# damien911224/ZeroShotVideoClassification

Hardware: AMD Instinct MI355X
Metric: clips/sec (fwd+bwd+step) R(2+1)D-18 16x112x112 bs=22/GPU (higher is better)
Workload: dtype f32; 1 GPU; r2plus1d_18 training step (zero_grad+fwd+MSE+bwd+Adam), 22 clips/GPU 3x16x112x112, random-init, fp32 (BASELINE.json configs[1]); clips_per_gpu=22, global_batch=22, optimizer=Adam lr=1e-3 (torch.optim.Adam), parallelism=dp1, world_size=1, launcher=single process, input=resident

## Files before the change

zeroshotvideoclassification_amd/csrc/conv_params.h:

```cpp
#pragma once
#include <hip/hip_runtime.h>
#include <stdint.h>
#include "zsv_hip.h"
#include "zsv_common.h"

namespace zsv {

struct IgemmParams {
    int M;
    int P;
    int K;
    int taps, nHW, nW, nT, nH;
    int cS, cHW, cW;
    int oS, oHW, oW;
    int stT, stH, stW, rT, rH, rW;
    int gC, gT, gH, gW, gS, gHW;
    int gsT, gsH, gsW, goT, goH, goW;
    int dir;
    int a_m_stride, a_c_stride;
    int k0T, k0H, k0W, tsT, tsH, tsW, kH, kW;
    unsigned g_bytes, a_bytes;
    int relu;
    int ksplit;
    int slab_elems;
    int lds_epilogue;
    float* stat_sum;
    float* stat_sq;
    int tiles_n;
    const float* pre_coef;
    int pre_pitch;
    int t2_cin;
    const float* acc_src;
};

inline bool t2_dense_shape(const zsv_conv_desc* d) {
    return d->kT == 3 && d->kH == 1 && d->kW == 1 && d->sT == 1 && d->sH == 1 && d->sW == 1 && d->pT == 1 && d->pH == 0 &&
           d->pW == 0 && d->Ti == 2 && d->To == 2 && d->Cin >= 16 && d->Cout >= 16;
}
inline zsv_conv_desc t2_dense_desc(const zsv_conv_desc* d) {
    zsv_conv_desc e = *d;
    e.Cin = 2 * d->Cin; e.Cout = 2 * d->Cout;
    e.Ti = e.To = 1; e.kT = 1; e.pT = 0;
    return e;
}
__host__ __device__ inline long t2_weight_offset(int co2, int c2, int cin) {
    return ((long)(co2 >> 1) * cin + (c2 >> 1)) * 3 + ((c2 & 1) - (co2 & 1) + 1);
}

enum { PANEL_NONE = 0, PANEL_LAUNCH_ONLY = 2, PANEL_RECORD = 3, PANEL_QUERY = 4 };
struct PanelCtx {
    int mode;
    void* ptr;
    size_t bytes;
    size_t need;
    int jobs;
    zsv_pack_job job;
};
extern thread_local PanelCtx g_panel;
inline bool panel_stop() { return g_panel.mode == PANEL_RECORD || g_panel.mode == PANEL_QUERY; }
inline bool panel_place(size_t need, void* workspace, float*& panel, int& st) {
    PanelCtx& pc = g_panel;
    st = ZSV_OK;
    panel = (float*)workspace;
    if (pc.mode == PANEL_QUERY) { pc.need = need; pc.jobs++; return false; }
    if (pc.mode != PANEL_NONE) {
        if (!pc.ptr || pc.bytes < need || (reinterpret_cast<uintptr_t>(pc.ptr) & 15) != 0) { st = ZSV_E_WORKSPACE; return false; }
        panel = (float*)pc.ptr;
    }
    return true;
}

template <int X> struct LdPad { static constexpr int value = (X % 32 == 16) ? X : X + 16; };

__device__ __forceinline__ int sgpr(int v) { return __builtin_amdgcn_readfirstlane(v); }


template <int TM, int TN>
__device__ __forceinline__ void store_tiles(const IgemmParams& prm, const f32x4 (&acc)[TM][TN], int m_base, int p_base,
                                            int lane, const float* __restrict__ bias, float* __restrict__ C) {
    const int frag_row = lane >> 4, frag_col = lane & 15;
#pragma unroll
    for (int j = 0; j < TN; ++j) {
        const int p = p_base + 16 * j + frag_col;
        if (p >= prm.P) continue;
        const int n = p / prm.cS;
        int r = p - n * prm.cS;
        const int ct = r / prm.cHW;
        r -= ct * prm.cHW;
        const int chh = r / prm.cW;
        const int cw = r - chh * prm.cW;
        const int sp = (ct * prm.stT + prm.rT) * prm.oHW + (chh * prm.stH + prm.rH) * prm.oW + cw * prm.stW + prm.rW;
        float* cbase = C + (size_t)n * prm.M * prm.oS + sp;
#pragma unroll
        for (int i = 0; i < TM; ++i) {
#pragma unroll
            for (int r4 = 0; r4 < 4; ++r4) {
                const int m = m_base + 16 * i + 4 * frag_row + r4;
                if (m < prm.M) {
                    float v = acc[i][j][r4];
                    if (prm.acc_src != nullptr) v += prm.acc_src[(cbase - C) + (size_t)m * prm.oS];
                    if (bias != nullptr) v += bias[m];
                    if (prm.relu) v = fmaxf(v, 0.f);
                    cbase[(size_t)m * prm.oS] = v;
                }
            }
        }
    }
}

template <int TM, int TN, int WGM, int WGN>
__device__ __forceinline__ void store_tiles_lds(const IgemmParams& prm, const f32x4 (&acc)[TM][TN], float* cs, int cap,
                                                int m0, int n0, int wave, int lane, const float* __restrict__ bias,
                                                float* __restrict__ C) {
    constexpr int BM = 16 * TM * WGM;
    constexpr int BN = 16 * TN * WGN;
    constexpr int PITCH = BN + 4;
    constexpr int RPI = 256 / BN == 0 ? 1 : 256 / BN;
    static_assert(BN == 128 || BN == 256, "read-back assumes 32 or 64 float4 per row");
    const int wm0 = (wave / WGN) * (16 * TM);
    const int wn0 = (wave % WGN) * (16 * TN);
    const int frag_row = lane >> 4, frag_col = lane & 15;
    int rp = (cap / PITCH) & ~15;
    if (rp > BM) rp = BM;
    const int c4 = BN == 128 ? (lane & 31) : lane;
    const int rsub = BN == 128 ? (lane >> 5) : 0;
    for (int r0 = 0; r0 < BM; r0 += rp) {
        __syncthreads();
#pragma unroll
        for (int i = 0; i < TM; ++i) {
            const int rb = wm0 + 16 * i - r0;
            if (rb >= 0 && rb < rp) {
#pragma unroll
                for (int j = 0; j < TN; ++j)
#pragma unroll
                    for (int r = 0; r < 4; ++r)
                        cs[(rb + 4 * frag_row + r) * PITCH + wn0 + 16 * j + frag_col] = acc[i][j][r];
            }
        }
        __syncthreads();
        const int rows = min(rp, BM - r0);
        const int p = n0 + 4 * c4;
        const bool pvalid = p < prm.P;
        const int n = pvalid ? p / prm.cS : 0;
        float* cbase = C + (size_t)n * prm.M * prm.oS + (p - n * prm.cS);
        f32x4 addn = {0.f, 0.f, 0.f, 0.f};
        auto fetch_add = [&](int rr) {
            const int m = m0 + r0 + rr;
            addn = f32x4{0.f, 0.f, 0.f, 0.f};
            if (pvalid && m < prm.M) addn = *reinterpret_cast<const f32x4*>(prm.acc_src + (cbase - C) + (size_t)m * prm.oS);
        };
        const bool has_add = prm.acc_src != nullptr;
        if (has_add && wave * RPI + rsub < rows) fetch_add(wave * RPI + rsub);
        for (int rr = wave * RPI + rsub; rr < rows; rr += 4 * RPI) {
            const int m = m0 + r0 + rr;
            f32x4 v = *reinterpret_cast<const f32x4*>(&cs[rr * PITCH + 4 * c4]);
            if (has_add) {
                v += addn;
                if (rr + 4 * RPI < rows) fetch_add(rr + 4 * RPI);
            }
            if (prm.stat_sum != nullptr) {
                float s1 = (v[0] + v[1]) + (v[2] + v[3]);
                float s2 = (v[0] * v[0] + v[1] * v[1]) + (v[2] * v[2] + v[3] * v[3]);
#pragma unroll
                for (int o = (BN == 128 ? 16 : 32); o > 0; o >>= 1) {
                    s1 += __shfl_xor(s1, o, 64);
                    s2 += __shfl_xor(s2, o, 64);
                }
                if (c4 == 0 && m < prm.M) {
                    const int tn = n0 / BN;
                    prm.stat_sum[(size_t)m * prm.tiles_n + tn] = s1;
                    prm.stat_sq[(size_t)m * prm.tiles_n + tn] = s2;
                }
            }
            if (pvalid && m < prm.M) {
                if (bias != nullptr) { const float b = bias[m]; v[0] += b; v[1] += b; v[2] += b; v[3] += b; }
                if (prm.relu) { v[0] = fmaxf(v[0], 0.f); v[1] = fmaxf(v[1], 0.f); v[2] = fmaxf(v[2], 0.f); v[3] = fmaxf(v[3], 0.f); }
                *reinterpret_cast<f32x4*>(cbase + (size_t)m * prm.oS) = v;
            }
        }
    }
}

__device__ __forceinline__ int xcd_tile(int nwg, int bid) {
    const int q = nwg >> 3, r = nwg & 7, xcd = bid & 7;
    return (xcd < r ? xcd * (q + 1) : r * (q + 1) + (xcd - r) * q) + (bid >> 3);
}

int igemm_generic(const IgemmParams& prm, bool avec, const float* A, const float* G, const float* bias, float* C,
                  hipStream_t stream);
bool igemm_tap_applicable(const IgemmParams& prm);
size_t igemm_tap_workspace_bytes(const IgemmParams& prm);
int igemm_tap(const IgemmParams& prm, const float* W, int w_m_stride, int w_c_stride, const float* G,
              const float* bias, float* C, void* workspace, size_t workspace_bytes, float* slabs, hipStream_t stream);
int igemm_tap_ksplit(const IgemmParams& prm);
int igemm_tap_stat_tiles(const IgemmParams& prm, const float* C);
int splitk_reduce(const float* slabs, int ksplit, long elems, int M, int oS, const float* bias, int relu, float* C,
                  hipStream_t stream);
int conv_check(const zsv_conv_desc* d);
size_t wgrad_generic_workspace_bytes(const zsv_conv_desc* d);
int wgrad_generic(const zsv_conv_desc* d, const float* x, const float* dy, float* dw, void* workspace,
                  size_t workspace_bytes, hipStream_t stream);
bool wino_dgrad_applicable(const zsv_conv_desc* d);
size_t wino_dgrad_workspace_bytes(const zsv_conv_desc* d);
int wino_dgrad(const zsv_conv_desc* d, const float* dy, const float* w, const float* add, float* dx, void* workspace,
               size_t workspace_bytes, hipStream_t stream);
bool dgrad_s2_applicable(const zsv_conv_desc* d);
size_t dgrad_s2_workspace_bytes(const zsv_conv_desc* d);
bool dgrad_s2_sub_supported(const zsv_conv_desc* d, int st, int sh, int sw);
int dgrad_s2(const zsv_conv_desc* d, const float* dy, const float* w, const float* sub, int sub_st, float* dx, void* workspace,
             size_t workspace_bytes, hipStream_t stream);
bool wino_fwd_applicable(const zsv_conv_desc* d);
bool wino_fwd_pre_capable(const zsv_conv_desc* d);
int wino_fwd_pre(const zsv_conv_desc* d, const float* x, const float* pre_coef, int pre_pitch, const float* w, float* stat_sum,
                 float* stat_sq, float* y, void* workspace, size_t workspace_bytes, hipStream_t stream);
bool wino_fwd_fusable(const zsv_conv_desc* d);
bool wino_dgrad_fusable(const zsv_conv_desc* d);
int wino_fwd_stat_tiles(const zsv_conv_desc* d);
size_t wino_fwd_workspace_bytes(const zsv_conv_desc* d);
int wino_fwd(const zsv_conv_desc* d, const float* x, const float* w, const float* bias, const float* residual, int relu,
             float* stat_sum, float* stat_sq, float* y, void* workspace, size_t workspace_bytes, hipStream_t stream);
bool wgrad_dma_applicable(const zsv_conv_desc* d, const float* x, const float* dy);
size_t wgrad_dma_workspace_bytes(const zsv_conv_desc* d);
int wgrad_dma(const zsv_conv_desc* d, const float* x, const float* dy, void* workspace, size_t workspace_bytes,
              int* slices_out, int* cpad_out, hipStream_t stream, const unsigned* vm_ext = nullptr);
int wgrad_vmask(const zsv_conv_desc* d, unsigned* out, hipStream_t stream);
bool wgrad_tring_applicable(const zsv_conv_desc* d, const float* x, const float* dy);
size_t wgrad_tring_workspace_bytes(const zsv_conv_desc* d);
int wgrad_tring_pre(const zsv_conv_desc* d, const float* x, const float* pre_coef, int pre_pitch, const float* dy, float* dw,
                    void* workspace, size_t workspace_bytes, hipStream_t stream);
int wgrad_tring(const zsv_conv_desc* d, const float* x, const float* dy, float* dw, void* workspace, size_t workspace_bytes,
                hipStream_t stream);
bool wgrad_wino_applicable(const zsv_conv_desc* d, const float* x, const float* dy);
size_t wgrad_wino_workspace_bytes(const zsv_conv_desc* d);
int wgrad_wino(const zsv_conv_desc* d, const float* x, const float* dy, float* dw, void* workspace, size_t workspace_bytes,
               hipStream_t stream, const unsigned* vm_ext = nullptr);

}
```

zeroshotvideoclassification_amd/csrc/conv_wgrad.hip:

```cpp
#include <hip/hip_runtime.h>
#include <stdint.h>
#include <stdlib.h>
#include "conv_params.h"
#include "knobs.h"

namespace zsv {

typedef float f32x2 __attribute__((ext_vector_type(2)));

struct WgradParams {
    int M;
    int Cin, Cpad, nblk;
    int taps, kHW, kW;
    int Kp;
    int P;
    int oS, oHW, oW;
    Magic m_oS, m_oHW, m_oW;
    int gT, gH, gW, gS, gHW, gCS;
    int sT, sH, sW, pT, pH, pW;
    int chunks_per_slice;
    unsigned x_bytes, dy_bytes;
};

template <int TM, int TN, int WGM, int WGN, bool AV4, int BP, bool TWOTAP>
__global__ __launch_bounds__(256, (BP == 16 ? 3 : 2)) void conv_wgrad_kernel(WgradParams prm, const float* __restrict__ X,
                                                         const float* __restrict__ DY,
                                                         float* __restrict__ OUT, int tiles_m, int tiles_mn) {
    constexpr int BM = 16 * TM * WGM;
    constexpr int BN = 16 * TN * WGN;
    constexpr int LDK = BP + 2;
    constexpr int NBLK = BN / 16;
    constexpr int RW = 64 / BP;
    constexpr int RPP = 4 * RW;
    constexpr int PB = 16 / RPP;
    constexpr int BPASS = NBLK * PB;
    constexpr int AQ = BP / 4;
    constexpr int ARP = 256 / AQ;
    constexpr int APASS = AV4 ? (BM + ARP - 1) / ARP : BM / RPP;
    constexpr unsigned OOB = 0xFFFFFFFFu;
    static_assert(WGM * WGN == 4, "4 waves");
    static_assert(BM % RPP == 0 || AV4, "tile rows must be a multiple of the staging pass");

    __shared__ __attribute__((aligned(16))) float As[2][BM * LDK];
    __shared__ float Bs[2][BN * LDK];

    const int tid = threadIdx.x;
    const int lane = tid & 63;
    const int wave = sgpr(tid >> 6);
    const int wm0 = (wave / WGN) * (16 * TM);
    const int wn0 = (wave % WGN) * (16 * TN);
    const int lin = xcd_tile(gridDim.x, blockIdx.x);
    const int tile = lin % tiles_mn;
    const int slice = lin / tiles_mn;
    const int m0 = (tile % tiles_m) * BM;
    const int n0 = (tile / tiles_m) * BN;

    const __amdgpu_buffer_rsrc_t x_rsrc = __builtin_amdgcn_make_buffer_rsrc(const_cast<float*>(X), 0, prm.x_bytes, 0x00020000);
    const __amdgpu_buffer_rsrc_t dy_rsrc = __builtin_amdgcn_make_buffer_rsrc(const_cast<float*>(DY), 0, prm.dy_bytes, 0x00020000);

    int b_kt[NBLK], b_kh[NBLK], b_kw[NBLK], b_ci0[NBLK];
    bool b_second[NBLK];
    bool has_tail = false;
    const int tap_first = min((n0 / 16) / prm.nblk, prm.taps - 1);
#pragma unroll
    for (int b = 0; b < NBLK; ++b) {
        const int blk = n0 / 16 + b;
        int tap = blk / prm.nblk;
        const int cb = blk - tap * prm.nblk;
        const bool live = tap < prm.taps;
        tap = live ? tap : 0;
        const int kt = tap / prm.kHW;
        const int r = tap - kt * prm.kHW;
        const int kh = r / prm.kW;
        b_kt[b] = kt; b_kh[b] = kh; b_kw[b] = r - kh * prm.kW;
        b_ci0[b] = live ? cb * 16 : prm.Cin;
        b_second[b] = live && tap != tap_first;
        has_tail = has_tail || (b_ci0[b] + 16 > prm.Cin);
    }
    int t2_kt[2], t2_kh[2], t2_kw[2];
#pragma unroll
    for (int q = 0; q < 2; ++q) {
        const int tap = min(tap_first + q, prm.taps - 1);
        t2_kt[q] = tap / prm.kHW;
        const int r = tap - t2_kt[q] * prm.kHW;
        t2_kh[q] = r / prm.kW;
        t2_kw[q] = r - t2_kh[q] * prm.kW;
    }

    const int pcol = tid & (BP - 1);
    const int half = (tid / BP) % RW;
    const int aq = tid % AQ, arow = tid / AQ;

    const int chunk_begin = slice * prm.chunks_per_slice;
    int chunk_end = chunk_begin + prm.chunks_per_slice;
    const int total_chunks = (prm.P + BP - 1) / BP;
    if (chunk_end > total_chunks) chunk_end = total_chunks;

    float breg[BPASS];
    f32x4 areg4[AV4 ? APASS : 1];
    float areg[AV4 ? 1 : APASS];
    const int ch_bytes = 4 * prm.gS;
    const int row_bytes = 4 * prm.oS;

    bool ld_pv = false;
    int ld_t0 = 0, ld_h0 = 0, ld_w0 = 0, ld_xb = 0;
    unsigned ld_dyb = OOB;
    unsigned ld_voff2[2] = {OOB, OOB};
    const float* ld_abase = DY;
    auto load_decode = [&](int chunk) {
        const unsigned p = (unsigned)(chunk * BP + pcol);
        ld_pv = p < (unsigned)prm.P;
        const unsigned n = mdiv(p, prm.m_oS);
        const unsigned r0 = p - n * prm.oS;
        const unsigned ot = mdiv(r0, prm.m_oHW);
        const unsigned r1 = r0 - ot * prm.oHW;
        const unsigned oh = mdiv(r1, prm.m_oW);
        const unsigned ow = r1 - oh * prm.oW;
        ld_t0 = (int)ot * prm.sT - prm.pT; ld_h0 = (int)oh * prm.sH - prm.pH; ld_w0 = (int)ow * prm.sW - prm.pW;
        ld_xb = 4 * ((int)n * prm.gCS + ld_t0 * prm.gHW + ld_h0 * prm.gW + ld_w0) + half * ch_bytes;
        if (TWOTAP) {
#pragma unroll
            for (int q = 0; q < 2; ++q) {
                const bool ok = ld_pv && (unsigned)(ld_t0 + t2_kt[q]) < (unsigned)prm.gT &&
                                (unsigned)(ld_h0 + t2_kh[q]) < (unsigned)prm.gH && (unsigned)(ld_w0 + t2_kw[q]) < (unsigned)prm.gW;
                ld_voff2[q] = ok ? (unsigned)(ld_xb + 4 * (t2_kt[q] * prm.gHW + t2_kh[q] * prm.gW + t2_kw[q])) : OOB;
            }
        }
        if (AV4) {
            unsigned p4 = (unsigned)(chunk * BP + 4 * aq);
            if (p4 + 4 > (unsigned)prm.P) p4 = (unsigned)prm.P - 4;
            const unsigned n4 = mdiv(p4, prm.m_oS);
            ld_abase = DY + (size_t)n4 * prm.M * prm.oS + (p4 - n4 * prm.oS);
        } else {
            ld_dyb = ld_pv ? 4u * (n * (unsigned)prm.M * (unsigned)prm.oS + r0) + (unsigned)(half * row_bytes) : OOB;
        }
    };
    auto load_b = [&](int b) {
        unsigned voff;
        if (TWOTAP) {
            voff = b_second[b] ? ld_voff2[1] : ld_voff2[0];
        } else {
            const bool ok = ld_pv && (unsigned)(ld_t0 + b_kt[b]) < (unsigned)prm.gT && (unsigned)(ld_h0 + b_kh[b]) < (unsigned)prm.gH &&
                            (unsigned)(ld_w0 + b_kw[b]) < (unsigned)prm.gW;
            voff = ok ? (unsigned)(ld_xb + 4 * (b_kt[b] * prm.gHW + b_kh[b] * prm.gW + b_kw[b])) : OOB;
        }
#pragma unroll
        for (int jj = 0; jj < PB; ++jj) {
            const int ci_u = b_ci0[b] + RW * wave + RPP * jj;
            unsigned v = voff;
            int soff = ci_u * ch_bytes;
            if (has_tail) {
                if (ci_u + half >= prm.Cin) v = OOB;
                if (ci_u >= prm.Cin) soff = 0;
            }
            breg[PB * b + jj] = __builtin_bit_cast(float, __builtin_amdgcn_raw_buffer_load_b32(x_rsrc, (int)v, soff, 0));
        }
    };
    auto load_a = [&](int j) {
        if (AV4) {
            int row = m0 + (arow + ARP * j) % BM;
            row = row < prm.M ? row : prm.M - 1;
            areg4[j] = *reinterpret_cast<const f32x4*>(ld_abase + (size_t)row * prm.oS);
        } else {
            const int row_u = m0 + RW * wave + RPP * j;
            unsigned v = (row_u + half < prm.M) ? ld_dyb : OOB;
            areg[j] = __builtin_bit_cast(float, __builtin_amdgcn_raw_buffer_load_b32(dy_rsrc, (int)v, row_u < prm.M ? row_u * row_bytes : 0, 0));
        }
    };
    auto load_part = [&](int chunk, int g, int ngp) {
        if (g == 0) load_decode(chunk);
#pragma unroll
        for (int b = 0; b < NBLK; ++b)
            if (b * ngp / NBLK == g) load_b(b);
#pragma unroll
        for (int j = 0; j < APASS; ++j)
            if (j * ngp / APASS == g) load_a(j);
    };
    auto load_chunk = [&](int chunk) {
#pragma unroll
        for (int g = 0; g < 4; ++g) load_part(chunk, g, 4);
    };

    auto store_chunk = [&](int buf) {
#pragma unroll
        for (int b = 0; b < NBLK; ++b)
#pragma unroll
            for (int jj = 0; jj < PB; ++jj)
                Bs[buf][(16 * b + RW * wave + half + RPP * jj) * LDK + pcol] = breg[PB * b + jj];
        if (AV4) {
#pragma unroll
            for (int j = 0; j < APASS; ++j) {
                float* dst = &As[buf][((arow + ARP * j) % BM) * LDK + 4 * aq];
                *reinterpret_cast<float2*>(dst) = make_float2(areg4[j][0], areg4[j][1]);
                *reinterpret_cast<float2*>(dst + 2) = make_float2(areg4[j][2], areg4[j][3]);
            }
        } else {
#pragma unroll
            for (int j = 0; j < APASS; ++j) As[buf][(RW * wave + half + RPP * j) * LDK + pcol] = areg[j];
        }
    };

    f32x4 acc[TM][TN];
#pragma unroll
    for (int i = 0; i < TM; ++i)
#pragma unroll
        for (int j = 0; j < TN; ++j) acc[i][j] = f32x4{0.f, 0.f, 0.f, 0.f};

    if (chunk_begin < chunk_end) {
        load_chunk(chunk_begin);
        store_chunk(0);
        if (chunk_begin + 1 < chunk_end) load_chunk(chunk_begin + 1);
    }
    __syncthreads();

    const int frag_k = lane >> 4;
    const int frag_r = lane & 15;
    constexpr int NG = BP / 8;
    for (int ch = chunk_begin; ch < chunk_end; ++ch) {
        const int cur = (ch - chunk_begin) & 1;
        if (ch + 1 < chunk_end) store_chunk(cur ^ 1);
        const int lchunk = min(ch + 2, chunk_end - 1);
        const float* as = &As[cur][0];
        const float* bs = &Bs[cur][0];
        float a[2][2][TM], b[2][2][TN];
        auto fetch = [&](int g, int slot) {
#pragma unroll
            for (int kk = 0; kk < 2; ++kk) {
#pragma unroll
                for (int i = 0; i < TM; ++i) a[slot][kk][i] = as[(wm0 + 16 * i + frag_r) * LDK + (2 * g + kk) * 4 + frag_k];
#pragma unroll
                for (int j = 0; j < TN; ++j) b[slot][kk][j] = bs[(wn0 + 16 * j + frag_r) * LDK + (2 * g + kk) * 4 + frag_k];
            }
        };
        fetch(0, 0);
#pragma unroll
        for (int g = 0; g < NG; ++g) {
            if (g + 1 < NG) fetch(g + 1, (g + 1) & 1);
            __builtin_amdgcn_sched_barrier(0);
            load_part(lchunk, g, NG);
#pragma unroll
            for (int kk = 0; kk < 2; ++kk)
#pragma unroll
                for (int i = 0; i < TM; ++i)
#pragma unroll
                    for (int j = 0; j < TN; ++j)
                        acc[i][j] = __builtin_amdgcn_mfma_f32_16x16x4f32(a[g & 1][kk][i], b[g & 1][kk][j], acc[i][j], 0, 0, 0);
            __builtin_amdgcn_sched_barrier(0);
        }
        __syncthreads();
    }

    float* out = OUT + (size_t)slice * prm.M * prm.Kp;
#pragma unroll
    for (int j = 0; j < TN; ++j) {
        const int k = n0 + wn0 + 16 * j + frag_r;
        if (k >= prm.Kp) continue;
#pragma unroll
        for (int i = 0; i < TM; ++i) {
#pragma unroll
            for (int r = 0; r < 4; ++r) {
                const int m = m0 + wm0 + 16 * i + 4 * frag_k + r;
                if (m < prm.M) out[(size_t)m * prm.Kp + k] = acc[i][j][r];
            }
        }
    }
}

__global__ __launch_bounds__(256) void slab_sum_kernel(const float* __restrict__ slabs, float* __restrict__ out,
                                                       int M, int Cin, int taps, int Cpad, int slices) {
    __shared__ float part[8][32];
    const size_t slab = (size_t)M * taps * Cpad;
    const int e = threadIdx.x & 31, g = threadIdx.x >> 5;
    for (size_t j0 = (size_t)blockIdx.x * 32; j0 < slab; j0 += (size_t)gridDim.x * 32) {
        const size_t j = j0 + e;
        const int ci = (int)(j % Cpad);
        const bool live = j < slab && ci < Cin;
        float s = 0.f;
        if (live) {
            const float* src = slabs + j;
            int k = g;
            for (; k + 24 < slices; k += 32) {
                const float v0 = src[(size_t)k * slab], v1 = src[(size_t)(k + 8) * slab];
                const float v2 = src[(size_t)(k + 16) * slab], v3 = src[(size_t)(k + 24) * slab];
                s += v0; s += v1; s += v2; s += v3;
            }
            for (; k < slices; k += 8) s += src[(size_t)k * slab];
        }
        part[g][e] = s;
        __syncthreads();
        if (g == 0 && live) {
            float t = part[0][e];
#pragma unroll
            for (int q = 1; q < 8; ++q) t += part[q][e];
            const size_t r = j / Cpad;
            const int tap = (int)(r % taps);
            const int co = (int)(r / taps);
            out[((size_t)co * Cin + ci) * taps + tap] = t;
        }
        __syncthreads();
    }
}

__global__ __launch_bounds__(256) void slab_sum_rows_kernel(const float* __restrict__ slabs, float* __restrict__ out,
                                                            int M, int Cin, int taps, int Cpad, int slices) {
    extern __shared__ __attribute__((aligned(16))) float row[];
    const int co = blockIdx.x;
    const int len = taps * Cpad;
    const size_t slab = (size_t)M * len;
    const float* src = slabs + (size_t)co * len;
    for (int i = 4 * (int)threadIdx.x; i < len; i += 1024) {
        f32x4 t = *reinterpret_cast<const f32x4*>(src + i);
        int k = 1;
        for (; k + 2 < slices; k += 3) {
            const f32x4 v0 = *reinterpret_cast<const f32x4*>(src + (size_t)k * slab + i);
            const f32x4 v1 = *reinterpret_cast<const f32x4*>(src + (size_t)(k + 1) * slab + i);
            const f32x4 v2 = *reinterpret_cast<const f32x4*>(src + (size_t)(k + 2) * slab + i);
            t += v0; t += v1; t += v2;
        }
        for (; k < slices; ++k) t += *reinterpret_cast<const f32x4*>(src + (size_t)k * slab + i);
        *reinterpret_cast<f32x4*>(row + i) = t;
    }
    __syncthreads();
    float* dst = out + (size_t)co * Cin * taps;
    const int n = Cin * taps;
    for (int o = (int)threadIdx.x; o < n; o += 256) {
        const int ci = o / taps, tap = o - ci * taps;
        dst[o] = row[tap * Cpad + ci];
    }
}

int slab_sum(const float* slabs, float* dw, int M, int Cin, int taps, int Cpad, int slices, hipStream_t stream) {
    const size_t row_bytes = (size_t)taps * Cpad * sizeof(float);
    if (slices <= 32 && (long)M * slices <= 16384 && row_bytes <= 64 * 1024 && (reinterpret_cast<uintptr_t>(slabs) & 15) == 0 && !ZSV_KNOB(NO_SLAB_SUM_ROWS)) {
        static const hipError_t attr = hipFuncSetAttribute((const void*)slab_sum_rows_kernel, hipFuncAttributeMaxDynamicSharedMemorySize, 64 * 1024);
        if (attr != hipSuccess) return ZSV_E_LAUNCH;
        hipLaunchKernelGGL(slab_sum_rows_kernel, dim3((unsigned)M), dim3(256), row_bytes, stream, slabs, dw, M, Cin, taps, Cpad, slices);
        return hipGetLastError() == hipSuccess ? ZSV_OK : ZSV_E_LAUNCH;
    }
    const long n = (long)M * taps * Cpad;
    long blocks = (n + 31) / 32;
    if (blocks > 8192) blocks = 8192;
    hipLaunchKernelGGL(slab_sum_kernel, dim3((unsigned)blocks), dim3(256), 0, stream, slabs, dw, M, Cin, taps, Cpad, slices);
    return hipGetLastError() == hipSuccess ? ZSV_OK : ZSV_E_LAUNCH;
}

static int wgrad_bp() { return 32; }

__global__ __launch_bounds__(256) void t2_fold_kernel(const float* __restrict__ dw2, float* __restrict__ dw, int Cout, int Cin) {
    const long n = (long)Cout * Cin;
    for (long i = (long)blockIdx.x * 256 + threadIdx.x; i < n; i += (long)gridDim.x * 256) {
        const long co = i / Cin, c = i - co * Cin;
        const float* r0 = dw2 + (2 * co) * (2L * Cin) + 2 * c;
        const float* r1 = r0 + 2L * Cin;
        const f32x2 a = *reinterpret_cast<const f32x2*>(r0), b = *reinterpret_cast<const f32x2*>(r1);
        dw[3 * i] = b[0];
        dw[3 * i + 1] = a[0] + b[1];
        dw[3 * i + 2] = a[1];
    }
}

struct WgradPlan {
    int cfg;
    int bm, bn;
    int tiles_m, tiles_n, slices, chunks_per_slice;
    int Cpad, nblk, Kp;
};

static double wgrad_slices(long tiles, long chunks, int bp, int bm, int bn, long& slices) {
    const long lds_bytes = (long)(bm + bn) * 34 * 4 * 2;
    long per_cu = (160L * 1024) / lds_bytes;
    if (per_cu > 4) per_cu = 4;
    if (per_cu < 1) per_cu = 1;
    const long resident = 256L * per_cu;
    long max_slices = (chunks * bp + 511) / 512;
    if (max_slices < 1) max_slices = 1;
    if (max_slices > 1024) max_slices = 1024;
    slices = 1;
    double best_eff = -1.0;
    for (long s = 1; s <= max_slices && tiles * s <= 4 * resident + tiles; ++s) {
        const long wgs = tiles * s;
        const long rounds = (wgs + resident - 1) / resident;
        const double eff = (double)wgs / (double)(rounds * resident) - 0.02 * (double)wgs / (double)resident;
        if (eff > best_eff + 1e-9) { best_eff = eff; slices = s; }
    }
    return best_eff;
}

static WgradPlan wgrad_plan(const zsv_conv_desc* d) {
    WgradPlan pl;
    const int M = d->Cout;
    const int taps = d->kT * d->kH * d->kW;
    pl.nblk = (d->Cin + 15) / 16;
    pl.Cpad = pl.nblk * 16;
    pl.Kp = taps * pl.Cpad;
    const long P = (long)d->N * d->To * d->Ho * d->Wo;
    const int bp = wgrad_bp();
    const long chunks = (P + bp - 1) / bp;
    const int bms[4] = {144, 128, 64, 80};
    const double pen_m[4] = {1.00, 1.00, 1.05, 1.08};
    const int bns[2] = {128, 64};
    const double pen_n[2] = {1.00, 1.10};
    int best_m = 0, best_n = 0;
    double best_w = 1e300;
    for (int i = 0; i < 4; ++i)
        for (int j = 0; j < 2; ++j) {
            const long tm = (M + bms[i] - 1) / bms[i], tn = (pl.Kp + bns[j] - 1) / bns[j];
            long sl;
            const double eff = wgrad_slices(tm * tn, chunks, bp, bms[i], bns[j], sl);
            const double w = (double)(tm * bms[i]) * (double)(tn * bns[j]) * pen_m[i] * pen_n[j] / (eff > 1e-3 ? eff : 1e-3);
            if (w < best_w * 0.999) { best_w = w; best_m = i; best_n = j; }
        }
    if (const char* e = ZSV_KNOB(WGRAD_CFG)) best_m = atoi(e) & 3;
    pl.cfg = best_m;
    pl.bm = bms[best_m];
    pl.bn = bns[best_n];
    if (const char* e = ZSV_KNOB(WGRAD_BN)) pl.bn = atoi(e) == 64 ? 64 : 128;
    pl.tiles_m = (M + pl.bm - 1) / pl.bm;
    pl.tiles_n = (pl.Kp + pl.bn - 1) / pl.bn;
    const long tiles = (long)pl.tiles_m * pl.tiles_n;
    long slices;
    wgrad_slices(tiles, chunks, bp, pl.bm, pl.bn, slices);
    const long max_slices = ((chunks * bp + 511) / 512) < 1 ? 1 : ((chunks * bp + 511) / 512 > 1024 ? 1024 : (chunks * bp + 511) / 512);
    if (const char* e = ZSV_KNOB(WGRAD_WGS)) slices = atol(e) / tiles;
    if (slices > max_slices) slices = max_slices;
    if (slices < 1) slices = 1;
    pl.chunks_per_slice = (int)((chunks + slices - 1) / slices);
    pl.slices = (int)((chunks + pl.chunks_per_slice - 1) / pl.chunks_per_slice);
    return pl;
}

template <int TM, int TN, int WGM, int WGN>
static void wgrad_launch(const WgradParams& p, bool av4, bool twotap, dim3 grid, hipStream_t stream, const float* x,
                         const float* dy, float* out, int tiles_m, int tiles_mn) {
#define ZSV_WG(A, T) hipLaunchKernelGGL((conv_wgrad_kernel<TM, TN, WGM, WGN, A, 32, T>), grid, dim3(256), 0, stream, p, x, dy, out, tiles_m, tiles_mn)
    if (av4) { if (twotap) ZSV_WG(true, true); else ZSV_WG(true, false); }
    else { if (twotap) ZSV_WG(false, true); else ZSV_WG(false, false); }
#undef ZSV_WG
}

static bool wgrad_two_taps(int taps, int nblk, int bn) {
    const int nb = bn / 16, total = taps * nblk;
    for (int b0 = 0; b0 < total; b0 += nb) {
        const int last = (b0 + nb - 1 < total ? b0 + nb - 1 : total - 1);
        if (last / nblk - b0 / nblk > 1) return false;
    }
    return true;
}

}

using namespace zsv;

static bool t2_dense(const zsv_conv_desc* d) { return t2_dense_shape(d) && !ZSV_KNOB(NO_T2_DENSE); }
static size_t t2_dw_bytes(const zsv_conv_desc* d) { return ((size_t)4 * d->Cout * d->Cin * sizeof(float) + 255) & ~(size_t)255; }

extern "C" size_t zsv_conv3d_wgrad_workspace_bytes(const zsv_conv_desc* d) {
    if (conv_check(d) != ZSV_OK) return 0;
    if (t2_dense(d)) {
        const zsv_conv_desc d2 = t2_dense_desc(d);
        return t2_dw_bytes(d) + zsv_conv3d_wgrad_workspace_bytes(&d2);
    }
    if (d->Cin < 16) return wgrad_generic_workspace_bytes(d);
    const WgradPlan pl = wgrad_plan(d);
    size_t need = (size_t)pl.slices * d->Cout * pl.Kp * sizeof(float);
    if (wgrad_dma_applicable(d, nullptr, nullptr)) {
        const size_t b = wgrad_dma_workspace_bytes(d);
        if (b > need) need = b;
    }
    if (wgrad_wino_applicable(d, nullptr, nullptr)) {
        const size_t b = wgrad_wino_workspace_bytes(d);
        if (b > need) need = b;
    }
    if (wgrad_tring_applicable(d, nullptr, nullptr)) {
        const size_t b = wgrad_tring_workspace_bytes(d);
        if (b > need) need = b;
    }
    return need;
}

extern "C" int zsv_conv3d_wgrad_pre(const zsv_conv_desc* d, const float* x, const float* pre_coef, int32_t coef_pitch,
                                    const float* dy, float* dw, void* workspace, size_t workspace_bytes, void* stream_) {
    int st = conv_check(d);
    if (st) return st;
    if (!x || !dy || !dw || !pre_coef) return ZSV_E_NULL;
    if (!zsv_conv3d_pre_supported(d) || coef_pitch < d->Cin || !wgrad_tring_applicable(d, x, dy)) return ZSV_E_UNSUPPORTED;
    if (!workspace || workspace_bytes < zsv_conv3d_wgrad_workspace_bytes(d)) return ZSV_E_WORKSPACE;
    return wgrad_tring_pre(d, x, pre_coef, coef_pitch, dy, dw, workspace, workspace_bytes, (hipStream_t)stream_);
}

static int wgrad_dispatch(const zsv_conv_desc* d, const float* x, const float* dy, float* dw, void* workspace, size_t workspace_bytes,
                          const unsigned* vm_ext, void* stream_);

extern "C" int zsv_conv3d_wgrad(const zsv_conv_desc* d, const float* x, const float* dy, float* dw,
                                void* workspace, size_t workspace_bytes, void* stream_) {
    return wgrad_dispatch(d, x, dy, dw, workspace, workspace_bytes, nullptr, stream_);
}

static bool wgrad_takes_mask(const zsv_conv_desc* d) {
    if (conv_check(d) != ZSV_OK || t2_dense(d) || d->Cin < 16) return false;
    if (wgrad_wino_applicable(d, nullptr, nullptr)) return true;
    if (wgrad_tring_applicable(d, nullptr, nullptr)) return false;
    return wgrad_dma_applicable(d, nullptr, nullptr);
}

extern "C" size_t zsv_conv3d_wgrad_mask_bytes(const zsv_conv_desc* d) {
    return d != nullptr && wgrad_takes_mask(d) ? sizeof(unsigned) * (size_t)d->Ti * d->Hi * d->Wi : 0;
}

extern "C" int zsv_conv3d_wgrad_mask(const zsv_conv_desc* d, void* mask, void* stream_) {
    if (d == nullptr || mask == nullptr) return ZSV_E_NULL;
    if (!wgrad_takes_mask(d)) return ZSV_E_UNSUPPORTED;
    return wgrad_vmask(d, (unsigned*)mask, (hipStream_t)stream_);
}

extern "C" int zsv_conv3d_wgrad_masked(const zsv_conv_desc* d, const float* x, const float* dy, float* dw, void* workspace,
                                       size_t workspace_bytes, const void* mask, void* stream_) {
    if (d == nullptr) return ZSV_E_NULL;
    return wgrad_dispatch(d, x, dy, dw, workspace, workspace_bytes, wgrad_takes_mask(d) ? (const unsigned*)mask : nullptr, stream_);
}

static int wgrad_dispatch(const zsv_conv_desc* d, const float* x, const float* dy, float* dw, void* workspace, size_t workspace_bytes,
                          const unsigned* vm_ext, void* stream_) {
    int st = conv_check(d);
    if (st) return st;
    if (!x || !dy || !dw) return ZSV_E_NULL;
    hipStream_t stream = (hipStream_t)stream_;
    if (t2_dense(d)) {
        const zsv_conv_desc d2 = t2_dense_desc(d);
        const size_t head = t2_dw_bytes(d);
        if (!workspace || workspace_bytes < head + zsv_conv3d_wgrad_workspace_bytes(&d2)) return ZSV_E_WORKSPACE;
        float* dw2 = (float*)workspace;
        st = zsv_conv3d_wgrad(&d2, x, dy, dw2, (char*)workspace + head, workspace_bytes - head, stream_);
        if (st) return st;
        long blocks = ((long)d->Cout * d->Cin + 255) / 256;
        if (blocks > 4096) blocks = 4096;
        hipLaunchKernelGGL(t2_fold_kernel, dim3((unsigned)blocks), dim3(256), 0, stream, dw2, dw, d->Cout, d->Cin);
        return hipGetLastError() == hipSuccess ? ZSV_OK : ZSV_E_LAUNCH;
    }
    if (d->Cin < 16) return wgrad_generic(d, x, dy, dw, workspace, workspace_bytes, stream);
    const WgradPlan pl = wgrad_plan(d);
    const size_t need = zsv_conv3d_wgrad_workspace_bytes(d);
    if (!workspace || workspace_bytes < need) return ZSV_E_WORKSPACE;
    if (wgrad_wino_applicable(d, x, dy)) return wgrad_wino(d, x, dy, dw, workspace, workspace_bytes, stream, vm_ext);
    if (wgrad_tring_applicable(d, x, dy)) return wgrad_tring(d, x, dy, dw, workspace, workspace_bytes, stream);
    if (wgrad_dma_applicable(d, x, dy)) {
        int slices = 0, cpad = 0;
        st = wgrad_dma(d, x, dy, workspace, workspace_bytes, &slices, &cpad, stream, vm_ext);
        if (st) return st;
        return slab_sum((const float*)workspace, dw, d->Cout, d->Cin, d->kT * d->kH * d->kW, cpad, slices, stream);
    }

    WgradParams p;
    p.M = d->Cout;
    p.Cin = d->Cin; p.Cpad = pl.Cpad; p.nblk = pl.nblk;
    p.taps = d->kT * d->kH * d->kW;
    p.kHW = d->kH * d->kW; p.kW = d->kW;
    p.Kp = pl.Kp;
    p.P = d->N * d->To * d->Ho * d->Wo;
    p.oS = d->To * d->Ho * d->Wo; p.oHW = d->Ho * d->Wo; p.oW = d->Wo;
    p.m_oS = make_magic((unsigned)p.oS); p.m_oHW = make_magic((unsigned)p.oHW); p.m_oW = make_magic((unsigned)p.oW);
    p.gT = d->Ti; p.gH = d->Hi; p.gW = d->Wi;
    p.gS = d->Ti * d->Hi * d->Wi; p.gHW = d->Hi * d->Wi; p.gCS = d->Cin * p.gS;
    p.sT = d->sT; p.sH = d->sH; p.sW = d->sW; p.pT = d->pT; p.pH = d->pH; p.pW = d->pW;
    p.chunks_per_slice = pl.chunks_per_slice;
    p.x_bytes = 4u * (unsigned)((long)d->N * d->Cin * p.gS);
    p.dy_bytes = 4u * (unsigned)((long)d->N * d->Cout * p.oS);

    const bool av4 = (p.oS % 4 == 0) && (p.P >= 4) && ((reinterpret_cast<uintptr_t>(dy) & 15) == 0);
    const bool twotap = wgrad_two_taps(p.taps, pl.nblk, pl.bn) && !ZSV_KNOB(WGRAD_NO_TWOTAP);
    const int tiles_mn = pl.tiles_m * pl.tiles_n;
    const dim3 grid((unsigned)(tiles_mn * pl.slices));
    float* out = (float*)workspace;
    if (pl.bn == 64) {
        switch (pl.cfg) {
            case 0: wgrad_launch<9, 1, 1, 4>(p, av4, twotap, grid, stream, x, dy, out, pl.tiles_m, tiles_mn); break;
            case 1: wgrad_launch<8, 1, 1, 4>(p, av4, twotap, grid, stream, x, dy, out, pl.tiles_m, tiles_mn); break;
            case 2: wgrad_launch<4, 1, 1, 4>(p, av4, twotap, grid, stream, x, dy, out, pl.tiles_m, tiles_mn); break;
            default: wgrad_launch<5, 1, 1, 4>(p, av4, twotap, grid, stream, x, dy, out, pl.tiles_m, tiles_mn); break;
        }
    } else
    switch (pl.cfg) {
        case 0: wgrad_launch<9, 2, 1, 4>(p, av4, twotap, grid, stream, x, dy, out, pl.tiles_m, tiles_mn); break;
        case 1: wgrad_launch<4, 4, 2, 2>(p, av4, twotap, grid, stream, x, dy, out, pl.tiles_m, tiles_mn); break;
        case 2: wgrad_launch<4, 2, 1, 4>(p, av4, twotap, grid, stream, x, dy, out, pl.tiles_m, tiles_mn); break;
        default: wgrad_launch<5, 2, 1, 4>(p, av4, twotap, grid, stream, x, dy, out, pl.tiles_m, tiles_mn); break;
    }
    if (hipGetLastError() != hipSuccess) return ZSV_E_LAUNCH;
    return slab_sum((const float*)workspace, dw, p.M, p.Cin, p.taps, pl.Cpad, pl.slices, stream);
}

extern "C" size_t zsv_linear_wgrad_workspace_bytes(int32_t rows, int32_t in_features, int32_t out_features) {
    zsv_conv_desc d = {rows, in_features, 1, 1, 1, out_features, 1, 1, 1, 1, 1, 1, 1, 1, 1, 0, 0, 0};
    return zsv_conv3d_wgrad_workspace_bytes(&d);
}

extern "C" int zsv_linear_wgrad(const float* x, const float* dy, float* dw, int32_t rows, int32_t in_features,
                                int32_t out_features, void* workspace, size_t workspace_bytes, void* stream) {
    zsv_conv_desc d = {rows, in_features, 1, 1, 1, out_features, 1, 1, 1, 1, 1, 1, 1, 1, 1, 0, 0, 0};
    return zsv_conv3d_wgrad(&d, x, dy, dw, workspace, workspace_bytes, stream);
}
```

zeroshotvideoclassification_amd/csrc/knobs.h:

```cpp
#pragma once

#define ZSV_KNOB_LIST(X) \
    X(NO_FUSED_STATS) \
    X(NO_BN_FUSION) \
    X(BF16_NO_SAME) \
    X(BF16_NO_TSAME) \
    X(BF16_NO_SAME64) \
    X(BF16_NO_SAME9) \
    X(BF16_SAME9_MIN_CHUNKS) \
    X(WINOT_NO_T32) \
    X(BF16_GROUP_OUTER) \
    X(BF16_NO_WGRAD) \
    X(BF16_NO_WGRAD_GATHER) \
    X(BF16_WGRAD_WGS) \
    X(NO_DGRAD_S2) \
    X(NO_DGRAD_S2T) \
    X(DGRAD_S2_BN) \
    X(DGRAD_S2_KS) \
    X(NO_DOWN_FUSION) \
    X(DGRAD_S2_NO_X4) \
    X(CONV_CFG) \
    X(NO_SPLITK) \
    X(TAP_KS) \
    X(SPLITK_THRESH) \
    X(NO_CFG5) \
    X(NO_TAP) \
    X(NO_LDS_EPILOGUE) \
    X(WGRAD_CFG) \
    X(WGRAD_BN) \
    X(WGRAD_WGS) \
    X(WGRAD_NO_TWOTAP) \
    X(NO_WGRAD_DMA) \
    X(WGRAD_DMA_TM) \
    X(WGRAD_DMA_TN) \
    X(WGRAD_DMA_SLICES) \
    X(WGRAD_LINEAR_WALK) \
    X(NO_STEM_WGRAD) \
    X(STEM_WGRAD_WGS) \
    X(WGRAD_TRING_RESIDENT) \
    X(WGRAD_TRING_SLICES) \
    X(NO_WGRAD_TRING) \
    X(NO_WGRAD_TWINO) \
    X(WGRAD_WINO_SLICES) \
    X(NO_WINO) \
    X(NO_WGRAD_WINO) \
    X(NO_WGRAD_WINO4) \
    X(WINO_MIN_TILES) \
    X(WINO_NO_SPLITK) \
    X(NO_WINOT) \
    X(WINOT_MIN_TILES) \
    X(BN_NT_MB) \
    X(BN_NO_MASKED_G) \
    X(WINOT_MAX_WASTE) \
    X(NO_WINO_FWD) \
    X(WINO_NO_F43) \
    X(WINOT_NO_F43) \
    X(WINO_NO_X4) \
    X(NO_SLAB_SUM_ROWS) \
    X(SPLITK_REDUCE_SCALAR) \
    X(NO_PACK_TILED) \
    X(NO_T2_DENSE) \
    X(WINO_NO_VW) \
    X(WINO_VW_MIN_WGS) \
    X(WINOT_GENERIC_EPILOGUE) \
    X(WINO_GENERIC_EPILOGUE)

namespace zsv {
enum KnobId {
#define ZSV_KNOB_ENUM(name) K_##name,
    ZSV_KNOB_LIST(ZSV_KNOB_ENUM)
#undef ZSV_KNOB_ENUM
    K_COUNT
};
extern const char* volatile g_knobs[K_COUNT];
}

#define ZSV_KNOB(name) (::zsv::g_knobs[::zsv::K_##name])
```

Baseline: 580.0 clips/s.

## Add row-ring weight-gradient kernel for stride-2 1x3x3 spatial convolutions

Adds a specialized weight-gradient kernel for 1x3x3 stride-2 spatial convs with input widths 56 or 28. It streams dy chunks and a ring of input rows into LDS through buffer-to-LDS DMA, reuses those input rows across kh taps, and accumulates all nine taps in registers using f32 MFMA. Partial results per slice are summed with the existing slab_sum. It is enabled by default and placed after the DMA path in dispatch, so it only replaces the generic fallback. The cost is a larger workspace and a new hand-scheduled kernel with inline asm LDS reads.

Result: no change. 580.4 clips/s (median of 4 runs) (+0.1%).

```diff
diff --git a/zeroshotvideoclassification_amd/csrc/conv_params.h b/zeroshotvideoclassification_amd/csrc/conv_params.h
--- a/zeroshotvideoclassification_amd/csrc/conv_params.h
+++ b/zeroshotvideoclassification_amd/csrc/conv_params.h
@@ -234,5 +234,9 @@
 size_t wgrad_wino_workspace_bytes(const zsv_conv_desc* d);
 int wgrad_wino(const zsv_conv_desc* d, const float* x, const float* dy, float* dw, void* workspace, size_t workspace_bytes,
                hipStream_t stream, const unsigned* vm_ext = nullptr);
-
-}
+bool wgrad_s2rows_applicable(const zsv_conv_desc* d, const float* x, const float* dy);
+size_t wgrad_s2rows_workspace_bytes(const zsv_conv_desc* d);
+int wgrad_s2rows(const zsv_conv_desc* d, const float* x, const float* dy, void* workspace, size_t workspace_bytes, int* slices_out,
+                 hipStream_t stream);
+
+}
diff --git a/zeroshotvideoclassification_amd/csrc/conv_wgrad.hip b/zeroshotvideoclassification_amd/csrc/conv_wgrad.hip
--- a/zeroshotvideoclassification_amd/csrc/conv_wgrad.hip
+++ b/zeroshotvideoclassification_amd/csrc/conv_wgrad.hip
@@ -475,6 +475,10 @@
         const size_t b = wgrad_tring_workspace_bytes(d);
         if (b > need) need = b;
     }
+    if (wgrad_s2rows_applicable(d, nullptr, nullptr)) {
+        const size_t b = wgrad_s2rows_workspace_bytes(d);
+        if (b > need) need = b;
+    }
     return need;
 }
 
@@ -549,6 +553,12 @@
         if (st) return st;
         return slab_sum((const float*)workspace, dw, d->Cout, d->Cin, d->kT * d->kH * d->kW, cpad, slices, stream);
     }
+    if (wgrad_s2rows_applicable(d, x, dy)) {
+        int slices = 0;
+        st = wgrad_s2rows(d, x, dy, workspace, workspace_bytes, &slices, stream);
+        if (st) return st;
+        return slab_sum((const float*)workspace, dw, d->Cout, d->Cin, 9, d->Cin, slices, stream);
+    }
 
     WgradParams p;
     p.M = d->Cout;
diff --git a/zeroshotvideoclassification_amd/csrc/conv_wgrad_s2rows.hip b/zeroshotvideoclassification_amd/csrc/conv_wgrad_s2rows.hip
--- /dev/null
+++ b/zeroshotvideoclassification_amd/csrc/conv_wgrad_s2rows.hip
@@ -0,0 +1,321 @@
+#include <hip/hip_runtime.h>
+#include <stdlib.h>
+
+#include <atomic>
+#include <utility>
+
+#include "conv_params.h"
+#include "zsv_common.h"
+#include "zsv_hip.h"
+#include "knobs.h"
+
+namespace zsv {
+
+struct S2RowsParams {
+    int M, Cin, Kp;
+    int T, Hi;
+    int cpf;
+    int oS;
+    int chunks_total, chunks_per_slice;
+    int tiles_m, tiles_mn;
+    unsigned x_bytes, dy_bytes;
+};
+
+template <int OFF>
+__device__ __forceinline__ void s2r_read32(float& dst, unsigned addr) {
+    asm volatile("ds_read_b32 %0, %1 offset:%2" : "=v"(dst) : "v"(addr), "n"(OFF) : "memory");
+}
+template <int BASE, int... S>
+__device__ __forceinline__ void s2r_read_seq(float* dst, unsigned addr, std::integer_sequence<int, S...>) {
+    (s2r_read32<BASE + 4 * S>(dst[S], addr), ...);
+}
+__device__ __forceinline__ void s2r_tie(float& v) { asm volatile("" : "+v"(v)); }
+template <int... S>
+__device__ __forceinline__ void s2r_tie_seq(float* v, std::integer_sequence<int, S...>) {
+    (s2r_tie(v[S]), ...);
+}
+template <int N, int... S>
+__device__ __forceinline__ void s2r_wait(float* v, std::integer_sequence<int, S...> q) {
+    asm volatile("s_waitcnt lgkmcnt(%0)" ::"n"(N) : "memory");
+    s2r_tie_seq(v, q);
+}
+
+template <int WI, int TM>
+__global__ __launch_bounds__(256, 2) void conv_wgrad_s2rows_kernel(S2RowsParams prm, const float* __restrict__ X,
+                                                                   const float* __restrict__ DY, float* __restrict__ OUT) {
+#if defined(__HIP_DEVICE_COMPILE__)
+    typedef __attribute__((address_space(3))) void* lds_ptr_t;
+    constexpr int WO = WI / 2;
+    constexpr int RPC = 28 / WO;
+    constexpr int NR = 2 * RPC + 1;
+    constexpr int R = 2 * NR;
+    constexpr int PPR = WI / 4;
+    constexpr int CP = WI == 56 ? 15 : 7;
+    constexpr int CHF = 4 * CP;
+    constexpr int G = (32 * CP + 63) / 64;
+    constexpr int SLOTB = G * 1024;
+    constexpr int BI = (NR * G + 3) / 4;
+    constexpr int AROWS = 32 * TM;
+    constexpr int AI = (AROWS * 7 + 63) / 64;
+    constexpr int AIW = (AI + 3) / 4;
+    constexpr int ABYTES = AI * 1024;
+    constexpr int B_OFF = 2 * ABYTES;
+    constexpr unsigned OOB = 0xFFFFFFF0u;
+    static_assert(WI == 56 || WI == 28, "row widths");
+    static_assert((TM - 1) * 16 * 112 + 28 < 65536 && 4 * 14 < 65536, "immediate offsets of the fragment reads");
+    extern __shared__ __attribute__((aligned(16))) unsigned char lds[];
+
+    const int tid = threadIdx.x, lane = tid & 63;
+    const int wave = sgpr(tid >> 6);
+    const int wm = wave >> 1, wn = wave & 1;
+    const int g = lane >> 4, r16 = lane & 15;
+    const int lin = xcd_tile(gridDim.x, blockIdx.x);
+    const int tile = lin % prm.tiles_mn, slice = lin / prm.tiles_mn;
+    const int m0 = (tile % prm.tiles_m) * AROWS;
+    const int c0 = (tile / prm.tiles_m) * 32;
+    const int gc0 = slice * prm.chunks_per_slice;
+    const int nq = min(prm.chunks_per_slice, prm.chunks_total - gc0);
+
+    const __amdgpu_buffer_rsrc_t x_rsrc = __builtin_amdgcn_make_buffer_rsrc(const_cast<float*>(X), 0, prm.x_bytes, 0x00020000);
+    const __amdgpu_buffer_rsrc_t dy_rsrc = __builtin_amdgcn_make_buffer_rsrc(const_cast<float*>(DY), 0, prm.dy_bytes, 0x00020000);
+
+    const int cpc = prm.T * prm.cpf;
+    int i_n = gc0 / cpc;
+    int i_q = gc0 - i_n * cpc;
+    int i_t = i_q / prm.cpf;
+    int i_c = i_q - i_t * prm.cpf;
+    int i_sb = 0;
+    bool i_new = true;
+
+    unsigned a_voff[AIW];
+#pragma unroll
+    for (int k = 0; k < AIW; ++k) {
+        const int P = 64 * (wave + 4 * k) + lane;
+        const int row = P / 7, pc = P - 7 * row;
+        a_voff[k] = (row < AROWS && m0 + row < prm.M) ? 4u * (unsigned)(row * prm.oS + 4 * pc) : OOB;
+    }
+    const int thw = prm.T * prm.Hi * WI;
+    unsigned b_voff[BI];
+#pragma unroll
+    for (int k = 0; k < BI; ++k) {
+        const int it = wave + 4 * k;
+        const int P = 64 * (it % G) + lane;
+        const int ch = P / CP, pc = P - CP * ch;
+        b_voff[k] = (ch < 32 && pc < PPR && c0 + ch < prm.Cin) ? 4u * (unsigned)(ch * thw + 4 * pc) : OOB;
+    }
+
+    auto issue = [&](int buf) {
+        const int a_soff = sgpr(4 * ((i_n * prm.M + m0) * prm.oS + 28 * i_q));
+#pragma unroll
+        for (int k = 0; k < AIW; ++k) {
+            const int j = wave + 4 * k;
+            if (j < AI)
+                __builtin_amdgcn_raw_ptr_buffer_load_lds(dy_rsrc, (lds_ptr_t)(lds + buf * ABYTES + j * 1024), 16, (int)a_voff[k], a_soff, 0, 0);
+        }
+        const int r0 = sgpr(2 * RPC * i_c - 1);
+        const int sb = sgpr(i_sb);
+        const bool fresh = sgpr(i_new ? 1 : 0) != 0;
+        const int x_frame = sgpr(4 * (((i_n * prm.Cin + c0) * prm.T + i_t) * prm.Hi * WI));
+#pragma unroll
+        for (int k = 0; k < BI; ++k) {
+            const int it = wave + 4 * k;
+            const int j = it / G, grp = it - j * G;
+            if (it < NR * G && (fresh || j > 0)) {
+                const int row = r0 + j;
+                const bool ok = (unsigned)row < (unsigned)prm.Hi;
+                int slot = sb + j;
+                slot = slot >= R ? slot - R : slot;
+                __builtin_amdgcn_raw_ptr_buffer_load_lds(x_rsrc, (lds_ptr_t)(lds + B_OFF + slot * SLOTB + grp * 1024), 16,
+                                                         (int)(ok ? b_voff[k] : OOB), ok ? x_frame + 4 * row * WI : 0, 0, 0);
+            }
+        }
+    };
+
+    const bool live = (m0 + wm * 16 * TM < prm.M) && (c0 + wn * 16 < prm.Cin);
+    const int wbase = RPC == 1 ? 7 * g : 7 * (g & 1);
+    const int jrow = RPC == 1 ? 0 : 2 * (g >> 1);
+    const bool edge = wbase == 0;
+    const unsigned lds_base = (unsigned)(size_t)(__attribute__((address_space(3))) unsigned char*)lds;
+    const unsigned a_lane = lds_base + 4u * (unsigned)((wm * 16 * TM + r16) * 28 + 7 * g);
+    const unsigned b_lane = lds_base + B_OFF + 4u * (unsigned)((wn * 16 + r16) * CHF + 2 * wbase) - 4u;
+
+    f32x4 acc[TM][9];
+#pragma unroll
+    for (int i = 0; i < TM; ++i)
+#pragma unroll
+        for (int j = 0; j < 9; ++j) acc[i][j] = f32x4{0.f, 0.f, 0.f, 0.f};
+
+    using seq7 = std::make_integer_sequence<int, 7>;
+    using seq15 = std::make_integer_sequence<int, 15>;
+    auto read_a = [&](float (&a)[TM][7], unsigned addr) {
+        s2r_read_seq<0>(a[0], addr, seq7{});
+        s2r_read_seq<1792>(a[1], addr, seq7{});
+        s2r_read_seq<3584>(a[2], addr, seq7{});
+        if constexpr (TM > 3) s2r_read_seq<5376>(a[TM > 3 ? 3 : 0], addr, seq7{});
+    };
+    auto mfma_phase = [&](const float (&a)[TM][7], float (&b)[15], int kh) {
+        b[0] = edge ? 0.f : b[0];
+        __builtin_amdgcn_s_setprio(1);
+#pragma unroll
+        for (int s = 0; s < 7; ++s)
+#pragma unroll
+            for (int i = 0; i < TM; ++i)
+#pragma unroll
+                for (int kw = 0; kw < 3; ++kw)
+                    acc[i][3 * kh + kw] = __builtin_amdgcn_mfma_f32_16x16x4f32(a[i][s], b[2 * s + kw], acc[i][3 * kh + kw], 0, 0, 0);
+        __builtin_amdgcn_s_setprio(0);
+    };
+    auto compute = [&](int buf, int sb) {
+        unsigned baddr[3];
+#pragma unroll
+        for (int kh = 0; kh < 3; ++kh) {
+            int sl = sb + jrow + kh;
+            sl = sl >= R ? sl - R : sl;
+            baddr[kh] = b_lane + (unsigned)(sl * SLOTB);
+        }
+        float a[TM][7], b0[15], b1[15];
+        read_a(a, a_lane + (unsigned)(buf * ABYTES));
+        s2r_read_seq<0>(b0, baddr[0], seq15{});
+        s2r_read_seq<0>(b1, baddr[1], seq15{});
+        __builtin_amdgcn_sched_barrier(0);
+        s2r_wait<15>(b0, seq15{});
+#pragma unroll
+        for (int i = 0; i < TM; ++i) s2r_tie_seq(a[i], seq7{});
+        mfma_phase(a, b0, 0);
+        __builtin_amdgcn_sched_barrier(0);
+        s2r_read_seq<0>(b0, baddr[2], seq15{});
+        __builtin_amdgcn_sched_barrier(0);
+        s2r_wait<15>(b1, seq15{});
+        mfma_phase(a, b1, 1);
+        __builtin_amdgcn_sched_barrier(0);
+        s2r_wait<0>(b0, seq15{});
+        mfma_phase(a, b0, 2);
+        __builtin_amdgcn_sched_barrier(0);
+    };
+
+    int sb_cur = 0;
+    for (int q = -1; q < nq; ++q) {
+        const int cur = q & 1;
+        const int sb_next = sgpr(i_sb);
+        if (q + 1 < nq) {
+            issue(cur ^ 1);
+            const bool endf = i_c + 1 == prm.cpf, endc = endf && i_t + 1 == prm.T;
+            i_sb += endf ? NR : 2 * RPC;
+            i_sb = i_sb >= R ? i_sb - R : i_sb;
+            i_new = endf;
+            i_c = endf ? 0 : i_c + 1;
+            i_t = endc ? 0 : (endf ? i_t + 1 : i_t);
+            i_q = endc ? 0 : i_q + 1;
+            i_n += endc ? 1 : 0;
+        }
+        if (q >= 0 && live) compute(cur, sb_cur);
+        sb_cur = sb_next;
+        asm volatile("s_waitcnt vmcnt(0)" ::: "memory");
+        __syncthreads();
+    }
+
+    if (live) {
+        float* out = OUT + (size_t)slice * prm.M * prm.Kp;
+        const int ci = c0 + wn * 16 + r16;
+#pragma unroll
+        for (int tap = 0; tap < 9; ++tap) {
+#pragma unroll
+            for (int i = 0; i < TM; ++i) {
+#pragma unroll
+                for (int r = 0; r < 4; ++r) {
+                    const int m = m0 + (wm * TM + i) * 16 + 4 * g + r;
+                    if (m < prm.M) out[(size_t)m * prm.Kp + tap * prm.Cin + ci] = acc[i][tap][r];
+                }
+            }
+        }
+    }
+#endif
+}
+
+static std::atomic<long> g_s2rows_launches{0};
+
+constexpr bool kS2RowsByDefault = true;
+
+bool wgrad_s2rows_applicable(const zsv_conv_desc* d, const float* x, const float* dy) {
+    if (ZSV_KNOB(NO_WGRAD_S2ROWS)) return false;
+    if (!kS2RowsByDefault && !ZSV_KNOB(WGRAD_S2ROWS)) return false;
+    if (d->kT != 1 || d->kH != 3 || d->kW != 3 || d->sT != 1 || d->sH != 2 || d->sW != 2 || d->pT != 0 || d->pH != 1 || d->pW != 1) return false;
+    if (d->Wi != 56 && d->Wi != 28) return false;
+    if (d->Hi % 2 != 0 || d->Ho != d->Hi / 2 || d->Wo != d->Wi / 2 || d->To != d->Ti) return false;
+    if ((d->Ho * d->Wo) % 28 != 0) return false;
+    if (d->Cin < 16 || d->Cin % 16 != 0 || d->Cout < 1) return false;
+    if ((long)d->N * d->Cin * d->Ti * d->Hi * d->Wi >= (1L << 29) || (long)d->N * d->Cout * d->To * d->Ho * d->Wo >= (1L << 29)) return false;
+    if (x != nullptr && ((reinterpret_cast<uintptr_t>(x) | reinterpret_cast<uintptr_t>(dy)) & 15) != 0) return false;
+    return true;
+}
+
+struct S2RowsPlan {
+    int tm, tiles_m, tiles_c, slices, chunks_per_slice, cpf;
+    long chunks;
+};
+
+static S2RowsPlan s2rows_plan(const zsv_conv_desc* d) {
+    S2RowsPlan pl;
+    const int nb = (d->Cout + 15) / 16;
+    const int pad3 = (nb + 5) / 6 * 6, pad4 = (nb + 7) / 8 * 8;
+    pl.tm = pad4 <= pad3 ? 4 : 3;
+    pl.tiles_m = (nb + 2 * pl.tm - 1) / (2 * pl.tm);
+    pl.tiles_c = (d->Cin + 31) / 32;
+    pl.cpf = d->Ho * d->Wo / 28;
+    pl.chunks = (long)d->N * d->To * pl.cpf;
+    const long tiles = (long)pl.tiles_m * pl.tiles_c;
+    long slices = 512 / tiles;
+    if (const char* e = ZSV_KNOB(WGRAD_S2ROWS_SLICES)) slices = atol(e);
+    const long max_slices = (pl.chunks + 7) / 8;
+    if (slices > max_slices) slices = max_slices;
+    if (slices > 1024) slices = 1024;
+    if (slices < 1) slices = 1;
+    pl.chunks_per_slice = (int)((pl.chunks + slices - 1) / slices);
+    pl.slices = (int)((pl.chunks + pl.chunks_per_slice - 1) / pl.chunks_per_slice);
+    return pl;
+}
+
+size_t wgrad_s2rows_workspace_bytes(const zsv_conv_desc* d) {
+    const S2RowsPlan pl = s2rows_plan(d);
+    return (size_t)pl.slices * d->Cout * 9 * d->Cin * sizeof(float);
+}
+
+template <int WI, int TM>
+static int s2rows_launch(const S2RowsParams& p, int wgs, hipStream_t stream, const float* x, const float* dy, float* out) {
+    constexpr int CP = WI == 56 ? 15 : 7;
+    constexpr int NR = 2 * (28 / (WI / 2)) + 1;
+    constexpr int LDS_BYTES = 2 * ((32 * TM * 7 + 63) / 64) * 1024 + 2 * NR * ((32 * CP + 63) / 64) * 1024;
+    static const hipError_t attr = hipFuncSetAttribute((const void*)conv_wgrad_s2rows_kernel<WI, TM>,
+                                                       hipFuncAttributeMaxDynamicSharedMemorySize, LDS_BYTES);
+    if (attr != hipSuccess) return ZSV_E_LAUNCH;
+    hipLaunchKernelGGL((conv_wgrad_s2rows_kernel<WI, TM>), dim3((unsigned)wgs), dim3(256), LDS_BYTES, stream, p, x, dy, out);
+    return launch_status();
+}
+
+int wgrad_s2rows(const zsv_conv_desc* d, const float* x, const float* dy, void* workspace, size_t workspace_bytes, int* slices_out,
+                 hipStream_t stream) {
+    const S2RowsPlan pl = s2rows_plan(d);
+    if (!workspace || workspace_bytes < wgrad_s2rows_workspace_bytes(d)) return ZSV_E_WORKSPACE;
+    S2RowsParams p;
+    p.M = d->Cout; p.Cin = d->Cin; p.Kp = 9 * d->Cin;
+    p.T = d->Ti; p.Hi = d->Hi;
+    p.cpf = pl.cpf;
+    p.oS = d->To * d->Ho * d->Wo;
+    p.chunks_total = (int)pl.chunks;
+    p.chunks_per_slice = pl.chunks_per_slice;
+    p.tiles_m = pl.tiles_m; p.tiles_mn = pl.tiles_m * pl.tiles_c;
+    p.x_bytes = 4u * (unsigned)((long)d->N * d->Cin * d->Ti * d->Hi * d->Wi);
+    p.dy_bytes = 4u * (unsigned)((long)d->N * d->Cout * p.oS);
+    const int wgs = p.tiles_mn * pl.slices;
+    float* out = (float*)workspace;
+    int st;
+    if (d->Wi == 56) st = pl.tm == 4 ? s2rows_launch<56, 4>(p, wgs, stream, x, dy, out) : s2rows_launch<56, 3>(p, wgs, stream, x, dy, out);
+    else st = pl.tm == 4 ? s2rows_launch<28, 4>(p, wgs, stream, x, dy, out) : s2rows_launch<28, 3>(p, wgs, stream, x, dy, out);
+    if (st == ZSV_OK) g_s2rows_launches.fetch_add(1, std::memory_order_relaxed);
+    *slices_out = pl.slices;
+    return st;
+}
+
+}
+
+extern "C" long zsv_debug_wgrad_s2rows_launches(void) { return zsv::g_s2rows_launches.load(std::memory_order_relaxed); }
diff --git a/zeroshotvideoclassification_amd/csrc/knobs.h b/zeroshotvideoclassification_amd/csrc/knobs.h
--- a/zeroshotvideoclassification_amd/csrc/knobs.h
+++ b/zeroshotvideoclassification_amd/csrc/knobs.h
@@ -36,6 +36,9 @@
     X(WGRAD_DMA_SLICES) \
     X(WGRAD_LINEAR_WALK) \
     X(NO_STEM_WGRAD) \
+    X(NO_WGRAD_S2ROWS) \
+    X(WGRAD_S2ROWS) \
+    X(WGRAD_S2ROWS_SLICES) \
     X(STEM_WGRAD_WGS) \
     X(WGRAD_TRING_RESIDENT) \
     X(WGRAD_TRING_SLICES) \
```
